# IGNF/MAESTRO

Hardware: AMD Instinct MI355X
Metric: MAE-pretrain tiles/sec (higher is better)
Workload: dtype bf16

## Files before the change

### include/maestro_hip.h

```cpp
#ifndef MAESTRO_HIP_H
#define MAESTRO_HIP_H
#include <stddef.h>
#include <stdint.h>
#ifdef __cplusplus
extern "C" {
#endif

const char* mh_last_error(void);
int mh_version(void);

#define MH_GEMM_OUT_F32 1
#define MH_GEMM_BIAS 2
#define MH_GEMM_GELU 4
#define MH_GEMM_RESIDUAL 8
#define MH_GEMM_DGELU 16
#define MH_GEMM_ATOMIC 32
#define MH_GEMM_COLSUM 64
#define MH_GEMM_AUX_DGELU 128
#define MH_GEMM_MULAUX 256
#define MH_GEMM_AUX_U8 1024
#define MH_GEMM_C8_E5M2 512
#define MH_GEMM_FP8_TILE_256 2048
#define MH_GEMM_FP8_TILE_128 4096
#define MH_GEMM_FP8_TILE_128D 8192
int mh_gemm_bf16(int layout, int M, int N, int K, const void* A, int lda, const void* B, int ldb, void* C, int ldc,
                 int flags, const float* bias, const float* res, int ldr, const void* aux_in, void* aux_out,
                 int ldaux, float* colsum, void* stream);

enum { MH_TILE_AUTO = -1, MH_TILE_REG_128 = 0, MH_TILE_DMA_256 = 1, MH_TILE_DMA_256x128 = 2, MH_TILE_DMA_128x256 = 3,
       MH_TILE_DMA_128 = 4, MH_TILE_DMA_128x4 = 5, MH_TILE_DMA_256_LOCKSTEP = 6, MH_TILE_PP_128 = 7,
       MH_TILE_PP_128_DIAG1 = 8, MH_TILE_PP_128_DIAG2 = 9, MH_TILE_PP_128_DIAG3 = 10,
       MH_TILE_PP_128_DIAG4 = 11, MH_TILE_PP_128_DIAG5 = 12,
       MH_TILE_REG_64 = 13, MH_TILE_REG_192 = 14,
       MH_TILE_SK_192 = 15, MH_TILE_SK_256 = 16,
       MH_TILE_SK_DMA_256 = 17  };
int mh_gemm_bf16_tile(int tile, int layout, int M, int N, int K, const void* A, int lda, const void* B, int ldb, void* C,
                      int ldc, int flags, const float* bias, const float* res, int ldr, const void* aux_in, void* aux_out,
                      int ldaux, float* colsum, void* stream);

long mh_gemm_sk_workspace(int tile, int grid);
int mh_gemm_bf16_sk(int tile, int layout, int M, int N, int K, const void* A, int lda, const void* B, int ldb, void* C, int ldc,
                    int flags, const float* bias, const float* res, int ldr, void* workspace, long workspace_bytes, int grid,
                    void* stream);

typedef struct MhGroupedGemm {
    const void* A; const void* B; void* C;
    int M, N, K, lda, ldb, ldc, reserved, accumulate;
} MhGroupedGemm;
int mh_gemm_grouped_tn(const MhGroupedGemm* table_device, int n_problems, const uint32_t* tile_queues, int queue_len,
                       void* stream);

enum { MH_FP8_E4M3 = 0, MH_FP8_E5M2 = 1 };
int mh_gemm_fp8(int M, int N, int K, const void* A8, int lda, int a_format, const void* B8, int ldb, void* C, int ldc,
                int flags, const float* descale_a, const float* descale_b, const float* bias, const float* res, int ldr,
                const void* aux_in, void* aux_out, int ldaux, float* colsum, void* c8, int ldc8, const float* c8_scale,
                float* c8_amax, void* stream);
#define MH_FP8_AMAX_SUBSLOTS 32
#define MH_FP8_AMAX_STRIDE 64
#define MH_FP8_AMAX_PITCH (MH_FP8_AMAX_SUBSLOTS * MH_FP8_AMAX_STRIDE)
typedef struct MhQuantJob {
    const void* src; void* dst; void* dst_t;
    long n;
    int rows, cols, slot, is_f32, format, reserved;
} MhQuantJob;
int mh_quant_batched(const MhQuantJob* jobs_device, const unsigned long* items_device, int n_items, const float* scale,
                     float* amax, int mode, void* stream);
int mh_fp8_update_scales(float* amax, float* scale, float* descale, int n, float format_max, int margin_log2, void* stream);
typedef struct MhTransposeJob { const void* src; void* dst; int rows, cols; } MhTransposeJob;
int mh_transpose_u8_batched(const MhTransposeJob* jobs_device, const unsigned long* items_device, int n_items, void* stream);

int mh_layernorm_fwd(const float* x, int x_L, int x_off, const float* gamma, const float* beta, void* y, int y_L,
                     int y_off, int y_is_f32, float* mean, float* rstd, int B, int n, int dim, float eps, void* stream);
int mh_layernorm_fwd_fp8(const float* x, int x_L, int x_off, const float* gamma, const float* beta, void* y, int y_L,
                         int y_off, float* mean, float* rstd, int B, int n, int dim, float eps, void* y8,
                         const float* y8_scale, float* y8_amax, void* stream);
int mh_layernorm_bwd(const void* dy, int dy_L, int dy_off, int dy_is_f32, const float* x, int x_L, int x_off,
                     const float* gamma, const float* mean, const float* rstd, const float* dres, float* dx,
                     void* dx_bf16, float* dgamma, float* dbeta, float* dcol, float* workspace, int B, int n, int dim,
                     void* stream);
long mh_layernorm_bwd_workspace(int rows, int dim);
int mh_layernorm_bwd_partial(const void* dy, int dy_L, int dy_off, int dy_is_f32, const float* x, int x_L, int x_off,
                             const float* gamma, const float* mean, const float* rstd, const float* dres, float* dx,
                             void* dx_bf16, float* workspace, int B, int n, int dim, void* stream);
#define MH_COLSUM_ROWS 16
typedef struct {
    const float* src;
    float* dst;
    int rows, cols, ld, reserved;
} MhColsumJob;
int mh_colsum_batched(const MhColsumJob* jobs_device, int n_jobs, const uint64_t* blocks_device, int n_blocks, void* stream);

int mh_attn_fwd(const void* qkv, void* out, float* lse, int B, int N, int H, int D, float scale, void* stream);
int mh_attn_bwd(const void* qkv, const void* out, const void* dout, const float* lse, float* delta, void* dqkv,
                int B, int N, int H, int D, float scale, void* stream);
int mh_patchify(const float* img, void* cols, float* target, int BD, int Ctot, int S, int P, int Kpad,
                const int* norm_bands, int n_norm_groups, int normalise, int rescale_elev, void* stream);
int mh_patchify_bands(const float* img, void* cols, float* target, int BD, int Csrc, int c0, int Ctot, int S, int P, int Kpad,
                      const int* norm_bands, int n_norm_groups, int normalise, int rescale_elev, void* stream);

int mh_groupnorm_stats(const float* y, float* partial, float* stats, int BD, int L, int E, float eps, void* stream);
int mh_groupnorm_partial_size(int BD, int L, int E);
int mh_embed_finish(const float* y, const float* stats, const float* gamma, const float* beta, const float* pos,
                    const float* date, int date_rows, int date_off, float* xg, int B, int D, int L, int E, int tok_off,
                    int Lgroup, void* stream);
int mh_embed_finish_bwd(const float* dxg, const float* y, const float* stats, const float* gamma, void* dyc,
                        float* dgamma, float* dbeta, float* sums, int B, int D, int L, int E, int tok_off, int Lgroup,
                        void* stream);
int mh_date_features(const int16_t* dates, const int16_t* ref_date, float* out, int B, int D, int rows, int row_off,
                     float fac, void* stream);
int mh_resize(const float* in, float* out, long planes, int Hin, int Win, int Hout, int Wout, int mode, void* stream);
int mh_dihedral(const void* in, void* out, const uint8_t* flags, int B, long planes, int S, int elem_bytes, void* stream);
int mh_rescale_elev(const float* img, float* out, int BD, int C, int S, void* stream);
int mh_depatchify(const float* patches, float* img, int BD, int C, int S, int P, void* stream);

int mh_mask_select(const float* noise, const uint8_t* struct_mask, int* visible_idx, int* masked_idx, int* inv,
                   uint8_t* mask, int B, int L, int k, void* stream);
int mh_gather_rows(const float* src, const int* idx, float* dst, int B, int src_L, int n_idx, int dim, int dst_L,
                   int dst_off, void* stream);
int mh_scatter_rows(const float* ddst, const int* idx, float* dsrc, int B, int src_L, int n_idx, int dim, int dst_L,
                    int dst_off, void* stream);
int mh_expand_rows(const float* src, const int* inv, float* dst, int B, int L, int n, int dim, void* stream);
// ... 58 lines not shown
```

### maestro_amd/csrc/gemm_dma.hip

```cpp
#include "gemm_ring.hpp"

#ifndef MH_DMA_PRIO
#define MH_DMA_PRIO 0
#endif
#if MH_DMA_PRIO == 0
#define MH_PRIO_UP() __builtin_amdgcn_s_setprio(1)
#define MH_PRIO_DOWN() __builtin_amdgcn_s_setprio(0)
#else
#define MH_PRIO_UP() ((void)0)
#define MH_PRIO_DOWN() ((void)0)
#endif

namespace {

template <class T, bool A_KMAJOR, bool B_KMAJOR, int CALLER, bool STAGGER>
__device__ __forceinline__ void gemm_dma_tile(const GemmParams& p, int tile_m, int tile_n, int kbeg, int kend,
                                              unsigned char* smem) {
    constexpr int S = T::S, PA = T::PA, PB = T::PB, NW = T::NW;
    static_assert(T::LDS_BYTES >= NW * 32 * 68 * 4, "the ring doubles as epilogue staging");
    const int m0 = tile_m * T::BM, n0 = tile_n * T::BN;
    const int nk = (kend - kbeg + BK - 1) / BK;

    const int w = __builtin_amdgcn_readfirstlane(threadIdx.x >> 6), l = threadIdx.x & 63;
    constexpr int MT = T::MT;
    const int wm = (w / T::WN) * (16 * MT), wn = (w % T::WN) * 64;

    const __amdgpu_buffer_rsrc_t ra_src = __builtin_amdgcn_make_buffer_rsrc((void*)p.A, (short)0, (int)p.a_bytes, 0x00020000);
    const __amdgpu_buffer_rsrc_t rb_src = __builtin_amdgcn_make_buffer_rsrc((void*)p.B, (short)0, (int)p.b_bytes, 0x00020000);
    int va[PA], vb[PB];
    piece_offsets<A_KMAJOR, T::BM, NW, PA>(p.lda, m0, w, l, va);
    piece_offsets<B_KMAJOR, T::BN, NW, PB>(p.ldb, n0, w, l, vb);
    const int a_step = A_KMAJOR ? BK * p.lda * 2 : BK * 2;
    const int b_step = B_KMAJOR ? BK * p.ldb * 2 : BK * 2;
    const int a_off0 = A_KMAJOR ? kbeg * p.lda * 2 : kbeg * 2;
    const int b_off0 = B_KMAJOR ? kbeg * p.ldb * 2 : kbeg * 2;

    auto issue = [&](int t) {
        unsigned char* slot = smem + (t % S) * T::STAGE_BYTES;
#pragma unroll
        for (int h = 0; h < PA; ++h)
            __builtin_amdgcn_raw_ptr_buffer_load_lds(ra_src, (lds_void*)(slot + (w + NW * h) * 1024), 16, va[h],
                                                     a_off0 + t * a_step, 0, 0);
#pragma unroll
        for (int h = 0; h < PB; ++h)
            __builtin_amdgcn_raw_ptr_buffer_load_lds(rb_src, (lds_void*)(slot + T::A_BYTES + (w + NW * h) * 1024), 16, vb[h],
                                                     b_off0 + t * b_step, 0, 0);
    };

    f32x4 acc[4][MT];
#pragma unroll
    for (int j = 0; j < 4; ++j)
#pragma unroll
        for (int i = 0; i < MT; ++i) acc[j][i] = (f32x4){0.f, 0.f, 0.f, 0.f};

    for (int t = 0; t < S - 1 && t < nk; ++t) issue(t);

    auto wait_step = [&](int step) {
        const int younger = min(S - 2, nk - 1 - step);
        if (younger >= 2) wait_vmcnt<2 * (PA + PB)>();
        else if (younger == 1) wait_vmcnt<PA + PB>();
        else wait_vmcnt<0>();
    };
    bf16x8 fa[MT], fb[4];
    auto load_step = [&](int t) {
        const unsigned char* ta = smem + (t % S) * T::STAGE_BYTES;
        const unsigned char* tb = ta + T::A_BYTES;
#pragma unroll
        for (int j = 0; j < 4; ++j) fb[j] = read_frag<B_KMAJOR, T::BN>(tb, wn + 16 * j);
#pragma unroll
        for (int i = 0; i < MT; ++i) fa[i] = read_frag<A_KMAJOR, T::BM>(ta, wm + 16 * i);
        __builtin_amdgcn_sched_barrier(0);
        if (t + S - 1 < nk) issue(t + S - 1);
        __builtin_amdgcn_sched_barrier(0);
    };
    auto math_step = [&]() {
#pragma unroll
        for (int i = 0; i < MT; ++i)
#pragma unroll
            for (int j = 0; j < 4; ++j)
                acc[j][i] = __builtin_amdgcn_mfma_f32_16x16x32_bf16(fb[j], fa[i], acc[j][i], 0, 0, 0);
    };

    if constexpr (NW == 8 && STAGGER) {
        wait_step(0);
        __builtin_amdgcn_s_barrier();
#if MH_DMA_PRIO == 1
        if (w >= 4) __builtin_amdgcn_s_setprio(1);
#endif
        if (w < 4) {
            for (int t = 0; t < nk; ++t) {
                load_step(t);
                __builtin_amdgcn_s_barrier();
                __builtin_amdgcn_sched_barrier(0);
                MH_PRIO_UP(); math_step(); MH_PRIO_DOWN();
                if (t + 1 < nk) wait_step(t + 1);
                __builtin_amdgcn_s_barrier();
                __builtin_amdgcn_sched_barrier(0);
            }
        } else {
            __builtin_amdgcn_s_barrier();
            __builtin_amdgcn_sched_barrier(0);
            for (int t = 0; t < nk; ++t) {
                load_step(t);
                if (t + 1 < nk) wait_step(t + 1);
                __builtin_amdgcn_s_barrier();
                __builtin_amdgcn_sched_barrier(0);
                MH_PRIO_UP(); math_step(); MH_PRIO_DOWN();
                if (t + 1 < nk) {
                    __builtin_amdgcn_s_barrier();
                    __builtin_amdgcn_sched_barrier(0);
                }
            }
        }
    } else {
        for (int t = 0; t < nk; ++t) {
            wait_step(t);
            __builtin_amdgcn_s_barrier();
            load_step(t);
            math_step();
        }
        __builtin_amdgcn_s_barrier();
    }

    float* st = reinterpret_cast<float*>(smem) + w * (32 * 68);
    if (p.flags & MH_GEMM_ATOMIC) gemm_epilogue_atomic<MT>(p, acc, st, m0 + wm, n0 + wn);
    else gemm_epilogue_store<MT>(p, acc, st, m0 + wm, n0 + wn);
}

template <class T, bool A_KMAJOR, bool B_KMAJOR, bool STAGGER>
__global__ __launch_bounds__(T::NT, T::MIN_WG) void gemm_dma_kernel(GemmParams p) {
    __shared__ __attribute__((aligned(16))) unsigned char smem[T::LDS_BYTES];
    const int nwg = p.tiles_m * p.tiles_n;
    const int id = xcd_remap(blockIdx.x, nwg);
    int tile_m, tile_n;
    raster_tile<4>(p, id, tile_m, tile_n);
    const int kbeg = blockIdx.y * p.k_per_split;
    gemm_dma_tile<T, A_KMAJOR, B_KMAJOR, 0, STAGGER>(p, tile_m, tile_n, kbeg, min(p.K, kbeg + p.k_per_split), smem);
}

typedef Tile<2, 4, 4> T256;
typedef Tile<2, 2, 3> T256x128;
typedef Tile<1, 4, 3> T128x256;
typedef Tile<1, 2, 4> T128;
typedef Tile<2, 2, 4, 4> T128q;

template <class T, bool STAGGER>
__global__ __launch_bounds__(T::NT) void gemm_dma_grouped_tn_kernel(const MhGroupedGemm* __restrict__ table, int n_problems,
                                                                    const uint32_t* __restrict__ queues, int queue_len) {
    __shared__ __attribute__((aligned(16))) unsigned char smem[T::LDS_BYTES];
    const uint32_t e = queues[(size_t)(blockIdx.x & 7) * queue_len + (blockIdx.x >> 3)];
    if (e == 0xFFFFFFFFu || (int)(e >> 16) >= n_problems) return;
    const MhGroupedGemm g = table[e >> 16];
    GemmParams p;
    p.A = (const bf16_t*)g.A; p.B = (const bf16_t*)g.B; p.C = g.C;
    p.bias = nullptr; p.res = nullptr; p.aux_in = nullptr; p.aux_out = nullptr; p.colsum = nullptr;
    p.M = g.M; p.N = g.N; p.K = g.K; p.lda = g.lda; p.ldb = g.ldb; p.ldc = g.ldc; p.ldr = 0; p.ldaux = 0;
    p.flags = MH_GEMM_OUT_F32 | (g.accumulate ? MH_GEMM_ATOMIC : 0);
    p.tiles_m = (g.M + T::BM - 1) / T::BM; p.tiles_n = (g.N + T::BN - 1) / T::BN; p.k_per_split = g.K; p.fast = 1;
    p.a_bytes = (unsigned)(((long)(g.K - 1) * g.lda + g.M) * 2);
    p.b_bytes = (unsigned)(((long)(g.K - 1) * g.ldb + g.N) * 2);
    const int tile_m = (e >> 8) & 0xff, tile_n = e & 0xff;
    if (tile_m >= p.tiles_m || tile_n >= p.tiles_n) return;
    gemm_dma_tile<T, true, true, 1, STAGGER>(p, tile_m, tile_n, 0, g.K, smem);
}

template <class T>
int launch_dma(int layout, GemmParams& p, hipStream_t s, bool stagger = true) {
    const int M = p.M, N = p.N, K = p.K;
    const bool a_kmajor = layout == 2, b_kmajor = layout != 0;
    p.tiles_m = ceil_div(M, T::BM); p.tiles_n = ceil_div(N, T::BN);
    const long a_reach = a_kmajor ? (long)(ceil_div(K, BK) * BK) * p.lda * 2 : (long)(p.tiles_m * T::BM) * p.lda * 2;
    const long b_reach = b_kmajor ? (long)(ceil_div(K, BK) * BK) * p.ldb * 2 : (long)(p.tiles_n * T::BN) * p.ldb * 2;
    if (a_reach + 65536 >= (1L << 31) || b_reach + 65536 >= (1L << 31)) return -2;
    int splits = 1;
    if (p.flags & MH_GEMM_ATOMIC) {
        const int tiles = p.tiles_m * p.tiles_n, ksteps = ceil_div(K, BK);
        const int slots = 256 * (T::LDS_BYTES > 80 * 1024 ? 1 : 2);
        splits = max(1, min(min(slots / max(tiles, 1), ksteps / 8), 32));
    }
    const int ksteps_per = ceil_div(ceil_div(K, BK), splits);
    p.k_per_split = ksteps_per * BK;
    splits = ceil_div(K, p.k_per_split);
    dim3 grid(p.tiles_m * p.tiles_n, splits), block(T::NT);
    if (T::NW == 8 && stagger) {
        switch (layout) {
            case 0: hipLaunchKernelGGL((gemm_dma_kernel<T, false, false, T::NW == 8>), grid, block, 0, s, p); break;
            case 1: hipLaunchKernelGGL((gemm_dma_kernel<T, false, true, T::NW == 8>), grid, block, 0, s, p); break;
            default: hipLaunchKernelGGL((gemm_dma_kernel<T, true, true, T::NW == 8>), grid, block, 0, s, p); break;
        }
        return 0;
    }
    switch (layout) {
        case 0: hipLaunchKernelGGL((gemm_dma_kernel<T, false, false, false>), grid, block, 0, s, p); break;
        case 1: hipLaunchKernelGGL((gemm_dma_kernel<T, false, true, false>), grid, block, 0, s, p); break;
        default: hipLaunchKernelGGL((gemm_dma_kernel<T, true, true, false>), grid, block, 0, s, p); break;
    }
    return 0;
}

}

extern "C" int mh_gemm_grouped_tn(const MhGroupedGemm* table_device, int n_problems, const uint32_t* tile_queues,
                                  int queue_len, void* stream) {
    MH_CHECK_ARG(table_device && tile_queues && n_problems > 0 && n_problems < 65536 && queue_len > 0,
                 "mh_gemm_grouped_tn: bad arguments");
    hipLaunchKernelGGL((gemm_dma_grouped_tn_kernel<T256, true>), dim3(8 * queue_len), dim3(T256::NT), 0, (hipStream_t)stream,
                       table_device, n_problems, tile_queues, queue_len);
    MH_LAUNCH_CHECK();
    return 0;
}

int gemm_dma_dispatch(int tile, int layout, int M, int N, int K, const void* A, int lda, const void* B, int ldb, void* C,
                      int ldc, int flags, const float* bias, const float* res, int ldr, const void* aux_in, void* aux_out,
                      int ldaux, float* colsum, void* stream) {
    const bool a_kmajor = layout == 2, b_kmajor = layout != 0;
    if ((!a_kmajor || !b_kmajor) && K % BK != 0) return -2;
    if (lda % 8 || ldb % 8) return -2;
    GemmParams p;
    p.A = (const bf16_t*)A; p.B = (const bf16_t*)B; p.C = C;
    p.bias = bias; p.res = res; p.aux_in = (const bf16_t*)aux_in; p.aux_out = (bf16_t*)aux_out; p.colsum = colsum;
    p.M = M; p.N = N; p.K = K; p.lda = lda; p.ldb = ldb; p.ldc = ldc; p.ldr = ldr; p.ldaux = ldaux; p.flags = flags;
    const long a_ext = a_kmajor ? ((long)(K - 1) * lda + M) * 2 : ((long)(M - 1) * lda + K) * 2;
    const long b_ext = b_kmajor ? ((long)(K - 1) * ldb + N) * 2 : ((long)(N - 1) * ldb + K) * 2;
    p.fast = 1; p.a_bytes = (unsigned)a_ext; p.b_bytes = (unsigned)b_ext;
    hipStream_t s = (hipStream_t)stream;
    int rc;
    switch (tile) {
        case MH_TILE_DMA_256: rc = launch_dma<T256>(layout, p, s); break;
        case MH_TILE_DMA_256x128: rc = launch_dma<T256x128>(layout, p, s); break;
        case MH_TILE_DMA_128x256: rc = launch_dma<T128x256>(layout, p, s); break;
        case MH_TILE_DMA_128: rc = launch_dma<T128>(layout, p, s); break;
        case MH_TILE_DMA_128x4: rc = launch_dma<T128q>(layout, p, s); break;
        case MH_TILE_DMA_256_LOCKSTEP: rc = launch_dma<T256>(layout, p, s, false); break;
        default: return -2;
    }
    if (rc) return rc;
    MH_LAUNCH_CHECK();
    return 0;
}
```

### maestro_amd/engine.py

```python

from __future__ import annotations

import contextlib
import gc
import os
import weakref
import time

import torch
from torch import nn

from maestro_amd import hip
from maestro_amd.layers.utils import draw_struct_masks

F32, BF16, I32, U8 = torch.float32, torch.bfloat16, torch.int32, torch.uint8
_NEVER = object()
_ROCTX = os.environ.get("MAESTRO_ROCTX", "0") == "1"
RING = 4
ALIGN = 64


class ParamStore:

    def __init__(self, ordered: list[tuple[str, nn.Parameter]], device) -> None:
        self.names, self.offset, self.params = [], {}, []
        off = 0
        for name, p in ordered:
            if id(p) in self.offset:
                continue
            self.names.append(name)
            self.offset[id(p)] = off
            self.params.append(p)
            off += (p.numel() + ALIGN - 1) // ALIGN * ALIGN
        self.total = off
        self.flat = torch.zeros(off, dtype=F32, device=device)
        self.grad_all = torch.zeros(off + ALIGN, dtype=F32, device=device)
        self.grad, self.extra = self.grad_all[:off], self.grad_all[off:]
        self.fresh = True
        self.half = torch.zeros(off, dtype=BF16, device=device)
        for p in self.params:
            o = self.offset[id(p)]
            view = self.flat[o: o + p.numel()].view(p.shape)
            view.copy_(p.data.to(device))
            p.data = view
            p.grad = self.grad[o: o + p.numel()].view(p.shape)
        self._version = None

    def g(self, p) -> torch.Tensor:
        o = self.offset[id(p)]
        return self.grad[o: o + p.numel()].view(p.shape)

    def h(self, p) -> torch.Tensor:
        o = self.offset[id(p)]
        return self.half[o: o + p.numel()].view(p.shape)

    def span(self, params) -> tuple[int, int]:
        offs = [self.offset[id(p)] for p in params]
        ends = [self.offset[id(p)] + (p.numel() + ALIGN - 1) // ALIGN * ALIGN for p in params]
        return min(offs), max(ends)

    def _versions(self):
        return self.flat._version, sum(p._version for p in self.params)

    def refresh_half(self, force: bool = False) -> bool:
        v = self._versions()
        if force or v != self._version:
            hip.cast_bf16(self.flat, self.half, self.total)
            self._version = v
            return True
        return False

    def mark_synced(self) -> None:
        self._version = self._versions()

    def flat_from(self, other: nn.Module, own: nn.Module) -> torch.Tensor:
        theirs = dict(other.named_parameters())
        out = torch.zeros_like(self.flat)
        seen = set()
        for name, p in own.named_parameters():
            if id(p) in self.offset and id(p) not in seen:
                seen.add(id(p))
                o = self.offset[id(p)]
                out[o: o + p.numel()].copy_(theirs[name].detach().reshape(-1), non_blocking=False)
        return out

    @contextlib.contextmanager
    def swapped(self, other_flat: torch.Tensor, repack=None):
        keep = self.flat.clone()
        self.flat.copy_(other_flat)
        self.refresh_half(force=True)
        if repack is not None:
            repack()
        try:
            yield
        finally:
            self.flat.copy_(keep)
            self.refresh_half(force=True)
            if repack is not None:
                repack()


class Stack:

    def __init__(self, eng: "MAEEngine", holder, Bn: int, N: int, tag: str) -> None:
        self.eng, self.t, self.Bn, self.N, self.tag = eng, holder, Bn, N, tag
        dim, mlp = holder.dim, holder.mlp_dim
        self.dim, self.mlp, self.H, self.Dh = dim, mlp, holder.heads, holder.dim_head
        self.inner = self.H * self.Dh
        self.depth = holder.depth
        M = self.M = Bn * N
        dev = eng.device
        e = lambda *s, dt=F32: torch.empty(*s, dtype=dt, device=dev)
        self.xs = [e(M, dim) for _ in range(2 * self.depth + 1)]
        self.saved = []
        for _ in range(self.depth):
            self.saved.append(dict(
                mean1=e(M), rstd1=e(M), mean2=e(M), rstd2=e(M), h1=e(M, dim, dt=BF16), qkv=e(M, 3 * self.inner, dt=BF16),
                o=e(M, self.inner, dt=BF16), lse=e(Bn * self.H * N), h2=e(M, dim, dt=BF16),
                hpre=e(M, mlp, dt=U8 if eng.aux_flag else BF16), act=e(M, mlp, dt=BF16)))
        for s in self.saved:
            s.update(gy16=e(M, dim, dt=BF16), gmid16=e(M, dim, dt=BF16), dh=e(M, mlp, dt=BF16),
                     dqkv=e(M, 3 * self.inner, dt=BF16))
        self.dxa, self.dxb = e(M, dim), e(M, dim)
        self.dx0_16 = e(M, dim, dt=BF16)
        self.dh2, self.do, self.delta = e(M, dim, dt=BF16), e(M, self.inner, dt=BF16), e(Bn * self.H * N)
        self.ln_ws = e(max(1, hip.layernorm_bwd_workspace(M, dim)))
        self.cs_rows = (M + 63) // 64
        self.cs_ws = e(self.cs_rows, mlp)
        self.ln_rows = hip.layernorm_bwd_workspace(M, dim) // (3 * dim)
        for s in self.saved:
            s.update(ws1=e(self.ln_rows, 3 * dim), ws2=e(self.ln_rows, 3 * dim), cs=e(self.cs_rows, mlp))
        plan = getattr(eng, "fp8", None)
        self.f8 = None
        if plan is not None and all(plan.eligible(k) for k in (dim, self.inner, mlp)):
            self.f8 = []
            for (attn, ff) in holder.layers:
                d = dict(h1=e(M, dim, dt=U8), o=e(M, self.inner, dt=U8), h2=e(M, dim, dt=U8), act=e(M, mlp, dt=U8),
                         s_h1=plan.add_activation(), s_o=plan.add_activation(), s_h2=plan.add_activation(),
                         s_act=plan.add_activation())
                for key, lin in (("qkv", attn.to_qkv), ("proj", attn.to_out[0]), ("fc1", ff.net[1]), ("fc2", ff.net[4])):
                    cache = eng._fp8_weights.get(id(lin.weight))
                    if cache is None:
                        off = eng.store.offset[id(lin.weight)]
                        w8, slot = plan.add_weight(lin.weight.data, off)
                        cache = eng._fp8_weights[id(lin.weight)] = (w8, slot, plan.add_transposed(w8, off))
                    d["w_" + key], d["sw_" + key], d["wt_" + key] = cache
                d["dgrad"] = plan.dgrad and all(d["wt_" + k] is not None for k in ("qkv", "proj", "fc1", "fc2"))
                if d["dgrad"]:
                    d.update(gy8=e(M, dim, dt=U8), mid8=e(M, dim, dt=U8), dh8=e(M, mlp, dt=U8), dqkv8=e(M, 3 * self.inner, dt=U8),
                             g_gy=plan.add_gradient(), g_mid=plan.add_gradient(), g_dh=plan.add_gradient(),
                             g_dqkv=plan.add_gradient())
                self.f8.append(d)

    @property
    def x0(self):
        return self.xs[0]

    @property
    def x_last(self):
        return self.xs[-1]

    @property
    def top16(self):
        return self.saved[-1]["gy16"] if self.depth else self.dx0_16

    def top_bias_grad(self):
        return self.eng.store.g(self.t.layers[-1][1].net[4].bias) if self.depth else None

    def forward(self, before_layer=None) -> None:
        eng, ps, M = self.eng, self.eng.store, self.M
        dim, mlp, inner = self.dim, self.mlp, self.inner
        for l, (attn, ff) in enumerate(self.t.layers):
            if before_layer is not None:
                before_layer(l)
            s, x_in, x_mid, x_out = self.saved[l], self.xs[2 * l], self.xs[2 * l + 1], self.xs[2 * l + 2]
            if self.f8 is not None:
                self._forward_layer_fp8(l, attn, ff, s, x_in, x_mid, x_out)
                continue
            proj = attn.to_out[0]
            hip.layernorm_fwd(x_in, M, 0, attn.norm.weight, attn.norm.bias, s["h1"], M, 0, s["mean1"], s["rstd1"], 1, M, dim)
            hip.gemm(hip.GEMM_NT, M, 3 * inner, dim, s["h1"], dim, ps.h(attn.to_qkv.weight), dim, s["qkv"], 3 * inner)
            hip.attn_fwd(s["qkv"], s["o"], s["lse"], self.Bn, self.N, self.H, self.Dh, attn.scale)
            hip.gemm(hip.GEMM_NT, M, dim, inner, s["o"], inner, ps.h(proj.weight), inner, x_mid, dim,
                     hip.OUT_F32 | hip.BIAS | hip.RESIDUAL, bias=proj.bias, res=x_in, ldr=dim)
            ln2, fc1, fc2 = ff.net[0], ff.net[1], ff.net[4]
            hip.layernorm_fwd(x_mid, M, 0, ln2.weight, ln2.bias, s["h2"], M, 0, s["mean2"], s["rstd2"], 1, M, dim)
            hip.gemm(hip.GEMM_NT, M, mlp, dim, s["h2"], dim, ps.h(fc1.weight), dim, s["act"], mlp,
                     hip.BIAS | hip.GELU | hip.AUX_DGELU | eng.aux_flag, bias=fc1.bias, aux_out=s["hpre"], ldaux=mlp)
            hip.gemm(hip.GEMM_NT, M, dim, mlp, s["act"], mlp, ps.h(fc2.weight), mlp, x_out, dim,
                     hip.OUT_F32 | hip.BIAS | hip.RESIDUAL, bias=fc2.bias, res=x_mid, ldr=dim)

    def _forward_layer_fp8(self, l, attn, ff, s, x_in, x_mid, x_out) -> None:
        eng, M, dim, mlp, inner = self.eng, self.M, self.dim, self.mlp, self.inner
        plan, f = eng.fp8, self.f8[l]
        proj, ln2, fc1, fc2 = attn.to_out[0], ff.net[0], ff.net[1], ff.net[4]
        hip.layernorm_fwd_fp8(x_in, M, 0, attn.norm.weight, attn.norm.bias, s["h1"], M, 0, s["mean1"], s["rstd1"], 1, M, dim,
                              f["h1"], plan.a_scale(f["s_h1"]), plan.a_amax(f["s_h1"]))
        hip.gemm_fp8(M, 3 * inner, dim, f["h1"], dim, f["w_qkv"], dim, s["qkv"], 3 * inner, plan.a_descale(f["s_h1"]),
                     plan.w_descale(f["sw_qkv"]))
        hip.attn_fwd(s["qkv"], s["o"], s["lse"], self.Bn, self.N, self.H, self.Dh, attn.scale)
        plan.quantize(s["o"], f["o"], f["s_o"])
        hip.gemm_fp8(M, dim, inner, f["o"], inner, f["w_proj"], inner, x_mid, dim, plan.a_descale(f["s_o"]),
                     plan.w_descale(f["sw_proj"]), flags=hip.OUT_F32 | hip.BIAS | hip.RESIDUAL, bias=proj.bias, res=x_in, ldr=dim)
        hip.layernorm_fwd_fp8(x_mid, M, 0, ln2.weight, ln2.bias, s["h2"], M, 0, s["mean2"], s["rstd2"], 1, M, dim, f["h2"],
                              plan.a_scale(f["s_h2"]), plan.a_amax(f["s_h2"]))
        hip.gemm_fp8(M, mlp, dim, f["h2"], dim, f["w_fc1"], dim, s["act"], mlp, plan.a_descale(f["s_h2"]),
                     plan.w_descale(f["sw_fc1"]), flags=hip.BIAS | hip.GELU | hip.AUX_DGELU | eng.aux_flag, bias=fc1.bias, aux_out=s["hpre"],
                     ldaux=mlp, c8=f["act"], ldc8=mlp, c8_scale=plan.a_scale(f["s_act"]), c8_amax=plan.a_amax(f["s_act"]))
        hip.gemm_fp8(M, dim, mlp, f["act"], mlp, f["w_fc2"], mlp, x_out, dim, plan.a_descale(f["s_act"]),
                     plan.w_descale(f["sw_fc2"]), flags=hip.OUT_F32 | hip.BIAS | hip.RESIDUAL, bias=fc2.bias, res=x_mid, ldr=dim)

    def reduce_jobs(self, lo: int = 0, hi: int | None = None) -> list:
        ps, dim, mlp, jobs = self.eng.store, self.dim, self.mlp, []
        for l in range(lo, self.depth if hi is None else hi):
            attn, ff = self.t.layers[l]
            s, ln2, fc1, proj = self.saved[l], ff.net[0], ff.net[1], attn.to_out[0]
            jobs.append((s["cs"], ps.g(fc1.bias), self.cs_rows, mlp, mlp))
            for ws, norm, bias in ((s["ws2"], ln2, ps.g(proj.bias)),
                                   (s["ws1"], attn.norm, ps.g(self.t.layers[l - 1][1].net[4].bias) if l > 0 else None)):
                flat = ws.view(-1)
                jobs.append((flat, ps.g(norm.weight), self.ln_rows, dim, 3 * dim))
                jobs.append((flat[dim:], ps.g(norm.bias), self.ln_rows, dim, 3 * dim))
                if bias is not None:
                    jobs.append((flat[2 * dim:], bias, self.ln_rows, dim, 3 * dim))
        return jobs

    def wgrad_problems(self, lo: int = 0, hi: int | None = None) -> list:
        ps, M = self.eng.store, self.M
        dim, mlp, inner = self.dim, self.mlp, self.inner
        out = []
        for l in range(lo, self.depth if hi is None else hi):
            attn, ff = self.t.layers[l]
            s, fc1, fc2, proj = self.saved[l], ff.net[1], ff.net[4], attn.to_out[0]
            out += [(s["gy16"], s["act"], ps.g(fc2.weight), dim, mlp, M, dim, mlp, mlp),
                    (s["dh"], s["h2"], ps.g(fc1.weight), mlp, dim, M, mlp, dim, dim),
                    (s["gmid16"], s["o"], ps.g(proj.weight), dim, inner, M, dim, inner, inner),
                    (s["dqkv"], s["h1"], ps.g(attn.to_qkv.weight), 3 * inner, dim, M, 3 * inner, dim, dim)]
        return out

    def backward(self, dx_out: torch.Tensor, hi: int | None = None, lo: int = 0, defer: bool = False, ready: bool = True):
        eng, ps, M = self.eng, self.eng.store, self.M
        dim, mlp, inner = self.dim, self.mlp, self.inner
        AT = hip.OUT_F32 | hip.ATOMIC
        cur = dx_out
        hi = self.depth if hi is None else hi
        cur16 = self.saved[hi - 1]["gy16"] if hi > 0 else self.dx0_16
        for l in reversed(range(lo, hi)):
            attn, ff = self.t.layers[l]
            s, x_in, x_mid = self.saved[l], self.xs[2 * l], self.xs[2 * l + 1]
            ln2, fc1, fc2 = ff.net[0], ff.net[1], ff.net[4]
            proj = attn.to_out[0]
            cur16, mid16, dh, dqkv = s["gy16"], s["gmid16"], s["dh"], s["dqkv"]
            mid = self.dxa if cur is not self.dxa else self.dxb
            nxt = self.dxa if mid is not self.dxa else self.dxb
            nxt16 = self.saved[l - 1]["gy16"] if l > 0 else self.dx0_16
            f = self.f8[l] if self.f8 is not None and self.f8[l]["dgrad"] else None
            plan = getattr(eng, "fp8", None)
            f8 = f is not None and plan.grad_ready
            if f is not None:
                plan.quantize_grad(cur16, f["gy8"], f["g_gy"])
            if f8:
                hip.gemm_fp8(M, mlp, dim, f["gy8"], dim, f["wt_fc2"], dim, dh, mlp, plan.g_descale(f["g_gy"]),
                             plan.w_descale(f["sw_fc2"]), flags=hip.MULAUX | hip.COLSUM | hip.C8_E5M2 | eng.aux_flag, a_format=hip.FP8_E5M2,
                             aux_in=s["hpre"], ldaux=mlp, colsum=s["cs"] if defer else self.cs_ws, c8=f["dh8"], ldc8=mlp,
                             c8_scale=plan.g_scale(f["g_dh"]), c8_amax=plan.g_amax(f["g_dh"]))
            else:
                hip.gemm(hip.GEMM_NN, M, mlp, dim, cur16, dim, ps.h(fc2.weight), mlp, dh, mlp, hip.MULAUX | hip.COLSUM | eng.aux_flag,
                         aux_in=s["hpre"], ldaux=mlp, colsum=s["cs"] if defer else self.cs_ws)
                if f is not None:
                    plan.quantize_grad(dh, f["dh8"], f["g_dh"])
            if not defer:
                hip.colsum(self.cs_ws, ps.g(fc1.bias), self.cs_rows, mlp, mlp)
                hip.gemm(hip.GEMM_TN, dim, mlp, M, cur16, dim, s["act"], mlp, ps.g(fc2.weight), mlp, AT)
# ... 1000 lines not shown
```

### maestro_amd/hip.py

```python

from __future__ import annotations

import ctypes
import os
from pathlib import Path

import torch

_LIB_PATH = Path(__file__).resolve().parent / "lib" / "libmaestro_hip.so"
_lib = None

GEMM_NT, GEMM_NN, GEMM_TN = 0, 1, 2
OUT_F32, BIAS, GELU, RESIDUAL, DGELU, ATOMIC, COLSUM, AUX_DGELU, MULAUX, C8_E5M2, AUX_U8 = 1, 2, 4, 8, 16, 32, 64, 128, 256, 512, 1024


class HipExtensionError(RuntimeError):
    pass


def lib() -> ctypes.CDLL:
    global _lib
    if _lib is None:
        if not _LIB_PATH.exists():
            raise HipExtensionError(
# ... 177 lines not shown
        if forced is not None:
            t = int(forced)
            if TILE_PP_128 < t <= TILE_PP_128 + 5 and os.environ.get("MH_ALLOW_DIAG_TILES") != "1":
                raise HipExtensionError(f"MH_GEMM_TILE={t} selects a diagnostic build of the ping-pong tile that writes wrong "
                                        "outputs (present only in a -DMH_DIAG_TILES library); set MH_ALLOW_DIAG_TILES=1 to run it on purpose")
            return t
        dma = os.environ.get("MH_GEMM_DMA", "")[:1]
        if os.environ.get("MH_GEMM_PP", "")[:1] == "0" and dma == "":
            return TILE_DMA_256 if _uses_dma(layout, M, N, K, flags) else TILE_REG_128
        if dma == "0":
            return TILE_REG_128
        lockstep = os.environ.get("MH_DMA_STAGGER", "")[:1] == "0"
        if (dma == "1" and layout != GEMM_TN and not (flags & ATOMIC)) or (lockstep and _uses_dma(layout, M, N, K, flags)):
            return TILE_DMA_256_LOCKSTEP if lockstep else TILE_DMA_256
        if _tuning and not (flags & ATOMIC):
            targs = list(args)
            targs[10], targs[17] = tflags, None
            tile = _tune_gemm(key, tuple(targs))
        else:
            tile = TILE_AUTO
    return tile


def _uses_192(layout, M, N, K, flags) -> bool:
    if layout == GEMM_TN or (flags & (COLSUM | ATOMIC)) or K < 1536 or K % 64 or _uses_dma(layout, M, N, K, flags):
        return False
    t128 = -(-M // 128) * -(-N // 128)
    return 512 < t128 <= 576 and -(-M // 192) * -(-N // 128) <= 512


def _uses_pp(layout, M, N, K, flags) -> bool:
    if os.environ.get("MH_GEMM_PP", "")[:1] == "0":
        return False
    served = flags in (0, BIAS | GELU | AUX_DGELU | AUX_U8, OUT_F32 | BIAS | RESIDUAL)
    if not served or layout == GEMM_TN or K % 64 or K < 512 or N % 128 or _uses_192(layout, M, N, K, flags):
        return False
    t128 = -(-M // 128) * -(-N // 128)
    if layout != GEMM_NT or t128 < 256:
        return False
    if flags & GELU:
        return t128 <= 2304
    return not _uses_dma(layout, M, N, K, flags) or (K < 1024 and t128 <= 8192)


def _auto_tile_name(layout, M, N, K, flags) -> int:
    if _uses_192(layout, M, N, K, flags):
        return TILE_REG_192
    if _uses_pp(layout, M, N, K, flags):
        return TILE_PP_128
    return TILE_DMA_256 if _uses_dma(layout, M, N, K, flags) else TILE_REG_128


def gemm(layout: int, M: int, N: int, K: int, A, lda: int, B, ldb: int, C, ldc: int, flags: int = 0, bias=None,
         res=None, ldr: int = 0, aux_in=None, aux_out=None, ldaux: int = 0, colsum=None, tile: int | None = None) -> None:
    args = (layout, M, N, K, A, lda, B, ldb, C, ldc, flags, bias, res, ldr, aux_in, aux_out, ldaux, colsum)
    explicit = tile is not None
    if _instep is not None and _instep.cand is not None and not explicit and not (flags & ATOMIC):
        key = (layout, M, N, K, flags & ~COLSUM)
        e0, e1 = _instep.open(key)
        e0.record()
        rc = _gemm_tile(_instep.cand, *args)
        if rc == -2:
            _instep.reject(key)
            rc = _gemm_tile(TILE_AUTO, *args)
        _check(rc, "mh_gemm_bf16_tile")
        e1.record()
        return
    if not explicit:
        tile = _pick_tile(layout, M, N, K, flags, args)
    ev = None
    if _timer is not None:
        named = tile if tile != TILE_AUTO else _auto_tile_name(layout, M, N, K, flags)
        if named in (TILE_REG_64, TILE_REG_192) and (layout == GEMM_TN or (flags & COLSUM)):
            named = TILE_REG_128
        ev = _timer.record(_TILE_NAME[named].format(_LAYOUT_NAME[layout]), 2.0 * M * N * K, (M, N, K))
        ev[0].record()
    rc = _gemm_tile(tile, *args)
    if rc == -2 and not explicit:
        pinned = os.environ.get("MH_GEMM_DMA", "")[:1] == "1" or os.environ.get("MH_GEMM_PP", "")[:1] == "0"
        rc = _gemm_tile(TILE_REG_128 if pinned else TILE_AUTO, *args)
    if rc == -2:
        raise HipExtensionError(f"mh_gemm_bf16_tile: problem ({M}, {N}, {K}) does not qualify for tile {tile}")
    _check(rc, "mh_gemm_bf16_tile")
    if ev is not None:
        ev[1].record()


def call(name: str, *args) -> None:
    conv = []
    for a in args:
        if a is None or isinstance(a, torch.Tensor):
            conv.append(ptr(a))
        else:
            conv.append(a)
    _check(getattr(lib(), name)(*conv, stream()), name)


def _hbm_call(kind: str, nbytes: float, name: str, *args) -> None:
    if _timer is None:
        return call(name, *args)
    e0, e1 = _timer.record_bytes(kind, nbytes)
    e0.record()
    call(name, *args)
    e1.record()


def _esz(t) -> int:
    return 0 if t is None else t.element_size()


def layernorm_fwd(x, x_L, x_off, gamma, beta, y, y_L, y_off, mean, rstd, B, n, dim, eps=1e-5):
    _hbm_call(f"ln_fwd<{dim}>", float(B) * n * dim * (4 + _esz(y)), "mh_layernorm_fwd", x, _I(x_L), _I(x_off), gamma, beta, y, _I(y_L),
              _I(y_off), _I(1 if y.dtype == torch.float32 else 0), mean, rstd, _I(B), _I(n), _I(dim), _F(eps))


def layernorm_fwd_fp8(x, x_L, x_off, gamma, beta, y, y_L, y_off, mean, rstd, B, n, dim, y8, y8_scale, y8_amax, eps=1e-5):
    call("mh_layernorm_fwd_fp8", x, _I(x_L), _I(x_off), gamma, beta, y, _I(y_L), _I(y_off), mean, rstd, _I(B), _I(n), _I(dim),
         _F(eps), y8, y8_scale, y8_amax)


def layernorm_bwd_workspace(rows, dim) -> int:
    f = lib().mh_layernorm_bwd_workspace
    f.restype = ctypes.c_long
    return int(f(_I(rows), _I(dim)))


def layernorm_bwd(dy, dy_L, dy_off, x, x_L, x_off, gamma, mean, rstd, dres, dx, dx_bf16, dgamma, dbeta, dcol, workspace,
                  B, n, dim):
    _hbm_call(f"ln_bwd<{dim}>", float(B) * n * dim * (_esz(dy) + 4 + _esz(dres) + 4 + _esz(dx_bf16)), "mh_layernorm_bwd", dy, _I(dy_L),
              _I(dy_off), _I(1 if dy.dtype == torch.float32 else 0), x, _I(x_L), _I(x_off), gamma, mean, rstd, dres, dx, dx_bf16,
              dgamma, dbeta, dcol, workspace, _I(B), _I(n), _I(dim))


def layernorm_bwd_partial(dy, dy_L, dy_off, x, x_L, x_off, gamma, mean, rstd, dres, dx, dx_bf16, workspace, B, n, dim):
    _hbm_call(f"ln_bwd<{dim}>", float(B) * n * dim * (_esz(dy) + 4 + _esz(dres) + 4 + _esz(dx_bf16)), "mh_layernorm_bwd_partial", dy,
              _I(dy_L), _I(dy_off), _I(1 if dy.dtype == torch.float32 else 0), x, _I(x_L), _I(x_off), gamma, mean, rstd, dres, dx,
              dx_bf16, workspace, _I(B), _I(n), _I(dim))


COLSUM_ROWS = 16


class _MhColsumJob(ctypes.Structure):
    _fields_ = [("src", ctypes.c_void_p), ("dst", ctypes.c_void_p), ("rows", ctypes.c_int), ("cols", ctypes.c_int),
                ("ld", ctypes.c_int), ("reserved", ctypes.c_int)]


class ColsumBatch:

    def __init__(self, jobs, device) -> None:
        if not jobs:
            raise HipExtensionError("ColsumBatch: no jobs")
        arr = (_MhColsumJob * len(jobs))()
        for i, (src, dst, rows, cols, ld) in enumerate(jobs):
            if src.dtype != torch.float32 or dst.dtype != torch.float32 or not src.is_cuda or not dst.is_cuda:
                raise HipExtensionError("ColsumBatch: f32 device tensors expected")
            if rows <= 0 or cols <= 0 or ld < cols or src.numel() < (rows - 1) * ld + cols or dst.numel() < cols:
                raise HipExtensionError(f"ColsumBatch job {i}: shape ({rows}, {cols}, ld {ld}) does not fit its buffers")
            arr[i] = _MhColsumJob(src.data_ptr(), dst.data_ptr(), rows, cols, ld, 0)
        self.keep = [t for job in jobs for t in job[:2]]
        self.table = torch.frombuffer(bytearray(bytes(arr)), dtype=torch.uint8).to(device)
        blocks = []
        for i, (_, _, rows, cols, _) in enumerate(jobs):
            if cols > 65535 * 256 or len(jobs) > 32767:
                raise HipExtensionError("ColsumBatch: too many jobs / columns for the work-item encoding")
            for cb in range(-(-cols // 256)):
# ... 505 lines not shown
```

Before: 1853.

## Fuse LayerNorm into residual GEMM epilogue with full-row 128x512 tile

Adds a GEMM kernel whose 128x512 tile covers the whole 512-wide row, so the epilogue can add bias and residual, store the fp32 stream, and compute the row LayerNorm (mean, rstd, bf16 output) in place. The bf16 forward path of the decoder stack (dim 512, large M) uses it for the attention projection plus LN2 and for fc2 plus the next layer's LN1, which removes the separate layernorm kernels and their re-read of x. In exchange it uses a fixed large tile with one workgroup per SM and no split along N, which may parallelise worse than the tuned GEMM tiles, and the epilogue adds LDS reductions and barriers.

```diff
diff --git a/include/maestro_hip.h b/include/maestro_hip.h
--- a/include/maestro_hip.h
+++ b/include/maestro_hip.h
@@ -37,6 +37,10 @@
 int mh_gemm_bf16_tile(int tile, int layout, int M, int N, int K, const void* A, int lda, const void* B, int ldb, void* C,
                       int ldc, int flags, const float* bias, const float* res, int ldr, const void* aux_in, void* aux_out,
                       int ldaux, float* colsum, void* stream);
+
+int mh_gemm_bf16_ln_fwd(int layout, int M, int N, int K, const void* A, int lda, const void* B, int ldb, const float* bias,
+                        const float* res, int ldr, float* x, int ldx, const float* gamma, const float* beta, void* h, int ldh,
+                        float* mean, float* rstd, float eps, void* stream);
 
 long mh_gemm_sk_workspace(int tile, int grid);
 int mh_gemm_bf16_sk(int tile, int layout, int M, int N, int K, const void* A, int lda, const void* B, int ldb, void* C, int ldc,
diff --git a/maestro_amd/csrc/gemm_dma.hip b/maestro_amd/csrc/gemm_dma.hip
--- a/maestro_amd/csrc/gemm_dma.hip
+++ b/maestro_amd/csrc/gemm_dma.hip
@@ -14,10 +14,9 @@
 namespace {
 
 template <class T, bool A_KMAJOR, bool B_KMAJOR, int CALLER, bool STAGGER>
-__device__ __forceinline__ void gemm_dma_tile(const GemmParams& p, int tile_m, int tile_n, int kbeg, int kend,
-                                              unsigned char* smem) {
+__device__ __forceinline__ void gemm_dma_mainloop(const GemmParams& p, int tile_m, int tile_n, int kbeg, int kend,
+                                                  unsigned char* smem, f32x4 (&acc)[4][T::MT]) {
     constexpr int S = T::S, PA = T::PA, PB = T::PB, NW = T::NW;
-    static_assert(T::LDS_BYTES >= NW * 32 * 68 * 4, "the ring doubles as epilogue staging");
     const int m0 = tile_m * T::BM, n0 = tile_n * T::BN;
     const int nk = (kend - kbeg + BK - 1) / BK;
 
@@ -47,7 +46,6 @@
                                                      b_off0 + t * b_step, 0, 0);
     };
 
-    f32x4 acc[4][MT];
 #pragma unroll
     for (int j = 0; j < 4; ++j)
 #pragma unroll
@@ -121,10 +119,20 @@
         }
         __builtin_amdgcn_s_barrier();
     }
-
+}
+
+template <class T, bool A_KMAJOR, bool B_KMAJOR, int CALLER, bool STAGGER>
+__device__ __forceinline__ void gemm_dma_tile(const GemmParams& p, int tile_m, int tile_n, int kbeg, int kend,
+                                              unsigned char* smem) {
+    constexpr int MT = T::MT;
+    static_assert(T::LDS_BYTES >= T::NW * 32 * 68 * 4, "the ring doubles as epilogue staging");
+    f32x4 acc[4][MT];
+    gemm_dma_mainloop<T, A_KMAJOR, B_KMAJOR, CALLER, STAGGER>(p, tile_m, tile_n, kbeg, kend, smem, acc);
+    const int w = __builtin_amdgcn_readfirstlane(threadIdx.x >> 6);
+    const int wm = (w / T::WN) * (16 * MT), wn = (w % T::WN) * 64;
     float* st = reinterpret_cast<float*>(smem) + w * (32 * 68);
-    if (p.flags & MH_GEMM_ATOMIC) gemm_epilogue_atomic<MT>(p, acc, st, m0 + wm, n0 + wn);
-    else gemm_epilogue_store<MT>(p, acc, st, m0 + wm, n0 + wn);
+    if (p.flags & MH_GEMM_ATOMIC) gemm_epilogue_atomic<MT>(p, acc, st, tile_m * T::BM + wm, tile_n * T::BN + wn);
+    else gemm_epilogue_store<MT>(p, acc, st, tile_m * T::BM + wm, tile_n * T::BN + wn);
 }
 
 template <class T, bool A_KMAJOR, bool B_KMAJOR, bool STAGGER>
@@ -238,3 +246,146 @@
     MH_LAUNCH_CHECK();
     return 0;
 }
+
+namespace {
+
+typedef Tile<1, 8, 3> T128x512;
+
+struct LnParams {
+    const float* gamma; const float* beta; bf16_t* h; float* mean; float* rstd; int ldh; float eps;
+};
+
+__device__ __forceinline__ void row_partial(float v, int i, float* buf) {
+    const int w = __builtin_amdgcn_readfirstlane(threadIdx.x >> 6), l = threadIdx.x & 63;
+    v += __shfl_xor(v, 16, 64);
+    v += __shfl_xor(v, 32, 64);
+    if (l < 16) buf[(16 * i + l) * 8 + w] = v;
+}
+__device__ __forceinline__ float row_total(int i, const float* buf) {
+    const int l = threadIdx.x & 63;
+    const f32x4 a = *reinterpret_cast<const f32x4*>(buf + (16 * i + (l & 15)) * 8);
+    const f32x4 b = *reinterpret_cast<const f32x4*>(buf + (16 * i + (l & 15)) * 8 + 4);
+    return ((a[0] + a[1]) + (a[2] + a[3])) + ((b[0] + b[1]) + (b[2] + b[3]));
+}
+__device__ __forceinline__ void lds_barrier() { asm volatile("s_waitcnt lgkmcnt(0)\n\ts_barrier" ::: "memory"); }
+
+template <bool B_KMAJOR>
+__global__ __launch_bounds__(T128x512::NT, 1) void gemm_ln_fwd_kernel(GemmParams p, LnParams q) {
+    __shared__ __attribute__((aligned(16))) unsigned char smem[T128x512::LDS_BYTES];
+    constexpr int MT = T128x512::MT;
+    const int tile_m = blockIdx.x;
+    f32x4 acc[4][MT];
+    gemm_dma_mainloop<T128x512, false, B_KMAJOR, 2, true>(p, tile_m, 0, 0, p.K, smem, acc);
+
+    const int w = __builtin_amdgcn_readfirstlane(threadIdx.x >> 6), l = threadIdx.x & 63, g = l >> 4, lm = l & 15;
+    const int m_base = tile_m * T128x512::BM;
+#pragma unroll
+    for (int j = 0; j < 4; ++j) {
+        const f32x4 b = *reinterpret_cast<const f32x4*>(p.bias + 64 * w + 16 * j + 4 * g);
+#pragma unroll
+        for (int i = 0; i < MT; ++i) acc[j][i] += b;
+    }
+    auto store_x = [&](int i) {
+        const int m = m_base + 16 * i + lm;
+        if (m < p.M) {
+#pragma unroll
+            for (int j = 0; j < 4; ++j)
+                *reinterpret_cast<f32x4*>(reinterpret_cast<float*>(p.C) + (size_t)m * p.ldc + 64 * w + 16 * j + 4 * g) = acc[j][i];
+        }
+    };
+    constexpr int IB = 4;
+#pragma unroll
+    for (int i0 = 0; i0 < MT; i0 += IB) {
+        f32x4 add[IB][4];
+#pragma unroll
+        for (int ii = 0; ii < IB; ++ii) {
+            const int m = min(m_base + 16 * (i0 + ii) + lm, p.M - 1);
+#pragma unroll
+            for (int j = 0; j < 4; ++j) add[ii][j] = *reinterpret_cast<const f32x4*>(p.res + (size_t)m * p.ldr + 64 * w + 16 * j + 4 * g);
+        }
+#pragma unroll
+        for (int ii = 0; ii < IB; ++ii)
+#pragma unroll
+            for (int j = 0; j < 4; ++j) acc[j][i0 + ii] += add[ii][j];
+#pragma unroll
+        for (int ii = 0; ii < IB; ++ii) store_x(i0 + ii);
+        __builtin_amdgcn_sched_barrier(0);
+    }
+    float* red = reinterpret_cast<float*>(smem);
+#pragma unroll
+    for (int i = 0; i < MT; ++i) {
+        float s = 0.f;
+#pragma unroll
+        for (int j = 0; j < 4; ++j) s += (acc[j][i][0] + acc[j][i][1]) + (acc[j][i][2] + acc[j][i][3]);
+        row_partial(s, i, red);
+    }
+    lds_barrier();
+    const bool stats = w == 0 && g == 0;
+#pragma unroll
+    for (int i = 0; i < MT; ++i) {
+        const float mu = row_total(i, red) * (1.f / 512);
+        const int m = m_base + 16 * i + lm;
+        if (stats && m < p.M) q.mean[m] = mu;
+        float s = 0.f;
+#pragma unroll
+        for (int j = 0; j < 4; ++j)
+#pragma unroll
+            for (int e = 0; e < 4; ++e) { acc[j][i][e] -= mu; s += acc[j][i][e] * acc[j][i][e]; }
+        row_partial(s, i, red + 128 * 8);
+    }
+    lds_barrier();
+    f32x4 gam[4], bet[4];
+#pragma unroll
+    for (int j = 0; j < 4; ++j) {
+        gam[j] = *reinterpret_cast<const f32x4*>(q.gamma + 64 * w + 16 * j + 4 * g);
+        bet[j] = *reinterpret_cast<const f32x4*>(q.beta + 64 * w + 16 * j + 4 * g);
+    }
+#pragma unroll
+    for (int i = 0; i < MT; ++i) {
+        const float rs = rsqrtf(row_total(i, red + 128 * 8) * (1.f / 512) + q.eps);
+        const int m = m_base + 16 * i + lm;
+        if (m >= p.M) continue;
+        if (stats) q.rstd[m] = rs;
+#pragma unroll
+        for (int j = 0; j < 4; ++j) {
+            f32x4 o;
+#pragma unroll
+            for (int e = 0; e < 4; ++e) o[e] = acc[j][i][e] * rs * gam[j][e] + bet[j][e];
+            *reinterpret_cast<u32x2*>(q.h + (size_t)m * q.ldh + 64 * w + 16 * j + 4 * g) = (u32x2){pack_bf2(o[0], o[1]), pack_bf2(o[2], o[3])};
+        }
+    }
+}
+
+}
+
+extern "C" int mh_gemm_bf16_ln_fwd(int layout, int M, int N, int K, const void* A, int lda, const void* B, int ldb,
+                                   const float* bias, const float* res, int ldr, float* x, int ldx, const float* gamma,
+                                   const float* beta, void* h, int ldh, float* mean, float* rstd, float eps, void* stream) {
+    MH_CHECK_ARG(layout == 0 || layout == 1, "mh_gemm_bf16_ln_fwd: layout %d (NT or NN only)", layout);
+    MH_CHECK_ARG(N == T128x512::BN, "mh_gemm_bf16_ln_fwd: N = %d, the full-row tile needs N = 512", N);
+    MH_CHECK_ARG(M > 0 && K > 0 && K % BK == 0, "mh_gemm_bf16_ln_fwd: M = %d, K = %d (K %% 32 == 0)", M, K);
+    MH_CHECK_ARG(A && B && bias && res && x && gamma && beta && h && mean && rstd, "mh_gemm_bf16_ln_fwd: null pointer");
+    MH_CHECK_ARG(lda >= K && ldb >= (layout == 0 ? K : N) && ldx >= N && ldh >= N && ldr >= N,
+                 "mh_gemm_bf16_ln_fwd: leading dimension too small");
+    MH_CHECK_ARG(lda % 8 == 0 && ldb % 8 == 0 && ldx % 4 == 0 && ldh % 4 == 0 && ldr % 4 == 0,
+                 "mh_gemm_bf16_ln_fwd: misaligned leading dimension");
+    MH_CHECK_ARG((uintptr_t)A % 16 == 0 && (uintptr_t)B % 16 == 0 && (uintptr_t)x % 16 == 0 && (uintptr_t)h % 8 == 0 &&
+                 (uintptr_t)bias % 16 == 0 && (uintptr_t)res % 16 == 0 && (uintptr_t)gamma % 16 == 0 && (uintptr_t)beta % 16 == 0,
+                 "mh_gemm_bf16_ln_fwd: misaligned pointer");
+    const long a_ext = ((long)(M - 1) * lda + K) * 2;
+    const long b_ext = layout == 1 ? ((long)(K - 1) * ldb + N) * 2 : ((long)(N - 1) * ldb + K) * 2;
+    const long a_reach = (long)ceil_div(M, T128x512::BM) * T128x512::BM * lda * 2;
+    MH_CHECK_ARG(a_reach + 65536 < (1L << 31) && b_ext + 65536 < (1L << 31), "mh_gemm_bf16_ln_fwd: operand over 2 GiB");
+    GemmParams p;
+    p.A = (const bf16_t*)A; p.B = (const bf16_t*)B; p.C = x;
+    p.bias = bias; p.res = res; p.aux_in = nullptr; p.aux_out = nullptr; p.colsum = nullptr;
+    p.M = M; p.N = N; p.K = K; p.lda = lda; p.ldb = ldb; p.ldc = ldx; p.ldr = ldr; p.ldaux = 0; p.flags = MH_GEMM_OUT_F32;
+    p.tiles_m = ceil_div(M, T128x512::BM); p.tiles_n = 1; p.k_per_split = K;
+    p.fast = 1; p.a_bytes = (unsigned)a_ext; p.b_bytes = (unsigned)b_ext;
+    const LnParams q{gamma, beta, (bf16_t*)h, mean, rstd, ldh, eps};
+    dim3 grid(p.tiles_m), block(T128x512::NT);
+    if (layout == 1) hipLaunchKernelGGL((gemm_ln_fwd_kernel<true>), grid, block, 0, (hipStream_t)stream, p, q);
+    else hipLaunchKernelGGL((gemm_ln_fwd_kernel<false>), grid, block, 0, (hipStream_t)stream, p, q);
+    MH_LAUNCH_CHECK();
+    return 0;
+}
diff --git a/maestro_amd/engine.py b/maestro_amd/engine.py
--- a/maestro_amd/engine.py
+++ b/maestro_amd/engine.py
@@ -102,6 +102,8 @@
 
 class Stack:
 
+    LN_FUSE_MIN_M = 128 * 256
+
     def __init__(self, eng: "MAEEngine", holder, Bn: int, N: int, tag: str) -> None:
         self.eng, self.t, self.Bn, self.N, self.tag = eng, holder, Bn, N, tag
         dim, mlp = holder.dim, holder.mlp_dim
@@ -109,6 +111,8 @@
         self.inner = self.H * self.Dh
         self.depth = holder.depth
         M = self.M = Bn * N
+        self.ln_fuse = (dim == 512 and self.inner % 32 == 0 and mlp % 32 == 0 and M >= self.LN_FUSE_MIN_M
+                        and os.environ.get("MAESTRO_DEC_LN_FUSE", "1") != "0")
         dev = eng.device
         e = lambda *s, dt=F32: torch.empty(*s, dtype=dt, device=dev)
         self.xs = [e(M, dim) for _ in range(2 * self.depth + 1)]
@@ -178,17 +182,29 @@
                 self._forward_layer_fp8(l, attn, ff, s, x_in, x_mid, x_out)
                 continue
             proj = attn.to_out[0]
-            hip.layernorm_fwd(x_in, M, 0, attn.norm.weight, attn.norm.bias, s["h1"], M, 0, s["mean1"], s["rstd1"], 1, M, dim)
+            if not (self.ln_fuse and l > 0):
+                hip.layernorm_fwd(x_in, M, 0, attn.norm.weight, attn.norm.bias, s["h1"], M, 0, s["mean1"], s["rstd1"], 1, M, dim)
             hip.gemm(hip.GEMM_NT, M, 3 * inner, dim, s["h1"], dim, ps.h(attn.to_qkv.weight), dim, s["qkv"], 3 * inner)
             hip.attn_fwd(s["qkv"], s["o"], s["lse"], self.Bn, self.N, self.H, self.Dh, attn.scale)
-            hip.gemm(hip.GEMM_NT, M, dim, inner, s["o"], inner, ps.h(proj.weight), inner, x_mid, dim,
-                     hip.OUT_F32 | hip.BIAS | hip.RESIDUAL, bias=proj.bias, res=x_in, ldr=dim)
             ln2, fc1, fc2 = ff.net[0], ff.net[1], ff.net[4]
-            hip.layernorm_fwd(x_mid, M, 0, ln2.weight, ln2.bias, s["h2"], M, 0, s["mean2"], s["rstd2"], 1, M, dim)
+            if self.ln_fuse:
+                hip.gemm_ln_fwd(hip.GEMM_NT, M, inner, s["o"], inner, ps.h(proj.weight), inner, proj.bias, x_in, dim, x_mid, dim,
+                                ln2.weight, ln2.bias, s["h2"], dim, s["mean2"], s["rstd2"])
+            else:
+                hip.gemm(hip.GEMM_NT, M, dim, inner, s["o"], inner, ps.h(proj.weight), inner, x_mid, dim,
+                         hip.OUT_F32 | hip.BIAS | hip.RESIDUAL, bias=proj.bias, res=x_in, ldr=dim)
+                hip.layernorm_fwd(x_mid, M, 0, ln2.weight, ln2.bias, s["h2"], M, 0, s["mean2"], s["rstd2"], 1, M, dim)
             hip.gemm(hip.GEMM_NT, M, mlp, dim, s["h2"], dim, ps.h(fc1.weight), dim, s["act"], mlp,
                      hip.BIAS | hip.GELU | hip.AUX_DGELU | eng.aux_flag, bias=fc1.bias, aux_out=s["hpre"], ldaux=mlp)
-            hip.gemm(hip.GEMM_NT, M, dim, mlp, s["act"], mlp, ps.h(fc2.weight), mlp, x_out, dim,
-                     hip.OUT_F32 | hip.BIAS | hip.RESIDUAL, bias=fc2.bias, res=x_mid, ldr=dim)
+            if self.ln_fuse and l + 1 < self.depth:
+                if before_layer is not None:
+                    before_layer(l + 1)
+                nxt, sn = self.t.layers[l + 1][0].norm, self.saved[l + 1]
+                hip.gemm_ln_fwd(hip.GEMM_NT, M, mlp, s["act"], mlp, ps.h(fc2.weight), mlp, fc2.bias, x_mid, dim, x_out, dim,
+                                nxt.weight, nxt.bias, sn["h1"], dim, sn["mean1"], sn["rstd1"])
+            else:
+                hip.gemm(hip.GEMM_NT, M, dim, mlp, s["act"], mlp, ps.h(fc2.weight), mlp, x_out, dim,
+                         hip.OUT_F32 | hip.BIAS | hip.RESIDUAL, bias=fc2.bias, res=x_mid, ldr=dim)
 
     def _forward_layer_fp8(self, l, attn, ff, s, x_in, x_mid, x_out) -> None:
         eng, M, dim, mlp, inner = self.eng, self.M, self.dim, self.mlp, self.inner
diff --git a/maestro_amd/hip.py b/maestro_amd/hip.py
--- a/maestro_amd/hip.py
+++ b/maestro_amd/hip.py
@@ -283,6 +283,18 @@
     if rc == -2:
         raise HipExtensionError(f"mh_gemm_bf16_tile: problem ({M}, {N}, {K}) does not qualify for tile {tile}")
     _check(rc, "mh_gemm_bf16_tile")
+    if ev is not None:
+        ev[1].record()
+
+
+def gemm_ln_fwd(layout: int, M: int, K: int, A, lda: int, B, ldb: int, bias, res, ldr: int, x, ldx: int, gamma, beta,
+                h, ldh: int, mean, rstd, eps: float = 1e-5) -> None:
+    ev = None
+    if _timer is not None:
+        ev = _timer.record(f"gemm_ln_fwd_kernel<128x512,{_LAYOUT_NAME[layout]}>", 2.0 * M * 512 * K, (M, 512, K))
+        ev[0].record()
+    call("mh_gemm_bf16_ln_fwd", _I(layout), _I(M), _I(512), _I(K), A, _I(lda), B, _I(ldb), bias, res, _I(ldr), x, _I(ldx),
+         gamma, beta, h, _I(ldh), mean, rstd, _F(eps))
     if ev is not None:
         ev[1].record()
 
```

New measurement: 1859, median of 4. About the same (+0.3%).
